# robin-karlsson0/pc-accumulation-lib

Hardware: AMD Instinct MI355X
Metric: Mpoints/s projected+accumulated and BEV frames/s @256x256; 1/2/4/8 GPU (higher is better)
Workload: dtype f64; 1 GPU; KITTI-360 single forward cam, 120k pts/frame, 200 m horizon (~201 live frames, 5169634 stored pts), one 256x256x21 BEV per integrated frame; points_per_frame=120000, bev_px=256, view_m=80

## Files before the change

pc-accumulation-lib_amd/csrc/pca_api.hip:

```cpp
#include <stdio.h>
#include <cmath>
#include "pca_common.h"

__global__ __launch_bounds__(256) void pca_fetch_block_kernel(const uint4 *src, uint4 *dst, int64_t n16)
{
    for (int64_t i = (int64_t)blockIdx.x * 256 + threadIdx.x; i < n16; i += (int64_t)gridDim.x * 256) dst[i] = src[i];
}

int pca_fetch_block(pca_ctx *ctx, const void *mapped_host, int64_t offset, void *dev, int64_t bytes, hipStream_t s)
{
    if (bytes <= 0) return 0;
    void *src = nullptr;
    PCA_CHECK(ctx, hipHostGetDevicePointer(&src, const_cast<void *>(mapped_host), 0));
    src = reinterpret_cast<char *>(src) + offset;
    const int64_t n16 = (bytes + 15) / 16;
    const int grid = (int)((n16 + 255) / 256 < 64 ? (n16 + 255) / 256 : 64);
    hipLaunchKernelGGL(pca_fetch_block_kernel, dim3(grid), dim3(256), 0, s, reinterpret_cast<const uint4 *>(src),
                       reinterpret_cast<uint4 *>(dev), n16);
    PCA_CHECK(ctx, hipGetLastError());
    return 0;
}

int pca_ctx_reserve_tiles(pca_ctx *ctx, int64_t tiles, hipStream_t s)
{
// ... 87 lines not shown
            double Mr[6], Mt[2];
            for (int r = 0; r < 2; ++r) {
                for (int c = 0; c < 3; ++c) Mr[3 * r + c] = now[4 * r] * inv[c] + now[4 * r + 1] * inv[3 + c] + now[4 * r + 2] * inv[6 + c];
                Mt[r] = now[4 * r + 3] - (Mr[3 * r] * m[3] + Mr[3 * r + 1] * m[7] + Mr[3 * r + 2] * m[11]);
            }
            const double tx = Mt[0] - prm->origin[0], ty = Mt[1] - prm->origin[1];
            q[0] = prm->R[0] * tx + prm->R[1] * ty + prm->dx;
            q[1] = prm->R[3] * tx + prm->R[4] * ty + prm->dy;
            for (int c = 0; c < 3; ++c) {
                Q[c] = prm->R[0] * Mr[c] + prm->R[1] * Mr[3 + c];
                Q[3 + c] = prm->R[3] * Mr[c] + prm->R[4] * Mr[3 + c];
            }
        }
        for (int k = 0; k < 6; ++k) if (!std::isfinite(Q[k])) return true;
        if (!std::isfinite(q[0]) || !std::isfinite(q[1])) return true;
        for (int axis = 0; axis < 2; ++axis)
            for (int side = 0; side < 2; ++side) {
                const double s = side ? -1.0 : 1.0;
                const double *row = Q + 3 * axis;
                if (cone) {
                    const double ua = s * (row[0] * cone[0] + row[1] * cone[1] + row[2] * cone[2] + q[axis]);
                    bool out = ua >= h;
                    for (int k = 0; k < 4 && out; ++k) {
                        const double *d = cone + 3 + 3 * k;
                        out = s * (row[0] * d[0] + row[1] * d[1] + row[2] * d[2]) >= 0.0;
                    }
                    if (out) return false;
                }
                if (box) {
                    const float *b = box + 6 * (size_t)f;
                    if (b[0] <= b[1] && b[2] <= b[3] && b[4] <= b[5]) {
                        double lo = s * q[axis];
                        for (int c = 0; c < 3; ++c) {
                            const double x0 = s * row[c] * (double)b[2 * c], x1 = s * row[c] * (double)b[2 * c + 1];
                            lo += x0 < x1 ? x0 : x1;
                        }
                        if (lo >= h) return false;
                    }
                }
            }
        return true;
    };
    int a = 0, b = F - 1;
    while (a <= b && !visible(a)) ++a;
    while (b >= a && !visible(b)) --b;
    if (a > b) { *first = -1; *last = -1; } else { *first = a; *last = b; }
    return 0;
}

int pca_bev_view_hint(pca_ctx *ctx, int slot0, int F, const double *then, const float *box, const double *cone, const double now[12],
                      const pca_bev_params *prm)
{
    if (!ctx) return -1;
    int first = 0, last = 0;
    if (pca_host_view_hull(F, then, box, cone, now, prm, &first, &last)) return -1;
    if (first == 0 && last == F - 1) return 0;
    if (first < 0) { first = 0; last = -1; }
    ctx->bin_first = slot0 + first; ctx->bin_end = slot0 + last + 1; ctx->bin_valid = true;
    return 1;
}

int pca_bev_bin_range(pca_ctx *ctx, int slot_first, int slot_last_plus1)
{
    if (!ctx) return -1;
    ctx->bin_first = slot_first; ctx->bin_end = slot_last_plus1; ctx->bin_valid = slot_last_plus1 >= slot_first;
    return 0;
}

static inline bool box_inside(double x, double y, double lo, double hi) { return lo < x && x < hi && lo < y && y < hi; }

int pca_host_ego_to_grid(const double *full, int F, const double R[9], double dx, double dy, double view, int px,
                         double *rows, int32_t *start)
{
    if (F < 2) { if (F == 1 && start) start[0] = 0; return 0; }
    const double h = 0.5 * view, lo = -h, pxd = (double)px, half_px = 0.5 * pxd;
    auto rot = [&](const double *p, double &x, double &y, double &z) {
        x = fma(R[2], p[2], fma(R[1], p[1], R[0] * p[0])) + dx;
        y = fma(R[5], p[2], fma(R[4], p[1], R[3] * p[0])) + dy;
        z = fma(R[8], p[2], fma(R[7], p[1], R[6] * p[0]));
    };
    auto emit = [&](int m, double x, double y, double z) {
        rows[3 * m + 0] = floor(x / view * pxd + half_px);
        rows[3 * m + 1] = floor(y / view * pxd + half_px);
        rows[3 * m + 2] = z;
    };
    int m = 0;
    double ax, ay, az, bx, by, bz;
    rot(full, ax, ay, az);
    bool a_in = box_inside(ax, ay, lo, h);
    for (int k = 0; k + 1 < F; ++k) {
        rot(full + 3 * (k + 1), bx, by, bz);
        const bool b_in = box_inside(bx, by, lo, h);
        start[k] = m;
        if (a_in) emit(m++, ax, ay, az);
        if (a_in != b_in) {
            double x0 = ax, y0 = ay, x1 = bx, y1 = by, xm = 0.0, ym = 0.0, gap = __builtin_huge_val();
            while (gap > 1e-4) {
                xm = 0.5 * (x0 + x1);
                ym = 0.5 * (y0 + y1);
                const bool p0_in = box_inside(x0, y0, lo, h), mid_in = box_inside(xm, ym, lo, h);
                if (mid_in == p0_in) { gap = sqrt((xm - x0) * (xm - x0) + (ym - y0) * (ym - y0)); x0 = xm; y0 = ym; }
                else { gap = sqrt((xm - x1) * (xm - x1) + (ym - y1) * (ym - y1)); x1 = xm; y1 = ym; }
            }
            emit(m++, xm, ym, az);
        }
        ax = bx; ay = by; az = bz; a_in = b_in;
// ... 131 lines not shown
```

pc-accumulation-lib_amd/csrc/pca_bev.hip:

```cpp
#include "pca_bev_common.h"
#include "pca_k1_body.h"
#include <cstdlib>
#include <mutex>

#define KEY_INVALID 0xffffffffu
#define TS 8
#define TCELLS (TS * TS)
#define NFK (2 * TCELLS)
#ifndef AB_THREADS
#define AB_THREADS 1024
#endif
#define MAX_G 512
#ifndef BIN_RUNR
#define BIN_RUNR 4
#endif
#ifndef BIN_WPE
#define BIN_WPE 4
#endif
#ifndef BIN_UNR
#define BIN_UNR 4
#endif
#ifndef BIN_REG_P
#define BIN_REG_P 12
#endif
#ifndef C_THREADS
#define C_THREADS 256
#endif
#define C_WAVES (C_THREADS / 64)
#define C_HIST_WAVES 4
#define RGB_CAP 4096
#define CONTIG_MIN 2560
#define HEAVY_MIN_DEFAULT 2560
#define FLAG_ROAD (1u << 24)
#define FLAG_DYNOBJ (1u << 25)

struct __attribute__((aligned(16))) RecF { double z; uint32_t iw; uint32_t cw; };
struct RecD { double z; double inten; uint32_t c; uint32_t fk; };

struct alignas(16) BevArgs {
    pca_store st;
    const double *intensity64;
    const int64_t *frame_off;
    int slot_begin, slot_split, slot_end;
    int64_t max_points;
    pca_bev_params prm;
    int n_pend;
    int write_back;
    int pend_slot_end[PCA_BEV_MAX_CHAIN];
    Mat34 pend_T[PCA_BEV_MAX_CHAIN];
    int tx, T, G;
    int Gr, Gp;
    int tile_mult;
    int heavy_min;
    int stagger;
    uint32_t *key;
    uint32_t *bh;
    uint32_t *boff;
    int Gk;
    int bin_first, bin_end;
    int k1_slot, k1_n;
    uint32_t *bh0;
    int split;
    uint32_t *heavy_hint;
    uint32_t heavy_hint_known;
    uint32_t *span_hint;
    uint32_t span_hint_known;
    int heavy_launched;
    uint32_t *heavy;
    void *recs;
    double *planes;
    uint16_t *planes_f16;
    double *extra;
    uint32_t *status;
    int dbg;
};
#define HQ_CLASSES 32
#define HQ_CURSOR 32
#define HQ_DONE 33
#define HQ_IDS 64

struct Window { int64_t lo, hi, sp, c_lo, c_hi; };

__device__ __forceinline__ int chunk_index(const BevArgs &a, int64_t lo, int64_t sp, int64_t chunk)
{
    (void)a; (void)lo; (void)sp; (void)chunk;
    return (int)blockIdx.x;
}
#define K1_SEG 4096
#define K1_RIDE 32
__device__ __forceinline__ int64_t window_end(const BevArgs &a)
{
    const int e = a.Gk ? a.k1_slot : a.slot_end;
    return a.frame_off[a.bin_end < e ? a.bin_end : e];
}
__device__ __forceinline__ int64_t window_begin(const BevArgs &a) { return a.frame_off[a.bin_first]; }
__device__ __forceinline__ Window chunk_of(const BevArgs &a, int &g)
{
    Window w;
    w.lo = window_begin(a);
    const int64_t hi0 = window_end(a);
    w.sp = (a.Gk && a.slot_split > a.k1_slot) ? hi0 : a.frame_off[a.slot_split];
    w.hi = (hi0 - w.lo > a.max_points) ? w.lo + a.max_points : hi0;
    const int G = a.G - a.Gk;
    const int64_t chunk = (w.hi - w.lo + G - 1) / G;
    g = chunk_index(a, w.lo, w.sp, chunk);
    const int c = g - a.Gk;
    w.c_lo = w.lo + (int64_t)c * chunk;
    w.c_hi = w.c_lo + chunk < w.hi ? w.c_lo + chunk : w.hi;
    if (w.c_lo > w.hi) w.c_lo = w.c_hi = w.hi;
    return w;
}
__host__ __device__ __forceinline__ int64_t seg_stride(int64_t n, int G) { return (n + G - 1) / G; }
__device__ __forceinline__ bool bev_split(const BevArgs &a, int64_t window_points)
{
    return a.split == 2 || (a.split == 1 && window_points <= (int64_t)(a.G - a.Gk) * BIN_REG_P * AB_THREADS);
}
__device__ __forceinline__ int table_pos(const BevArgs &a, int g) { return a.Gp ? (g & 7) * a.Gp + (g >> 3) : g; }
__device__ __forceinline__ int table_group(const BevArgs &a, int p)
{
    if (!a.Gp) return p;
// ... 796 lines not shown
        const uint32_t other = dpp_or<0xb1>(0u, val);
        if (ok && !upper) L.S.med2[set][cell][ch] = val + other;
    }
}

__device__ __forceinline__ void wave_cells_hist(TileLds &L, const uint32_t *s_rgb)
{
    const int lane = threadIdx.x & 63, wave = threadIdx.x >> 6;
    if (wave >= C_HIST_WAVES) return;
    uint32_t *h = &L.whist[wave][0][0][0];
    for (int i = 0; i < TCELLS / C_HIST_WAVES; ++i) {
        const int cell = C_HIST_WAVES * i + wave;
        const uint32_t n_p = L.S.cnt[2 * cell], n_f = L.S.cnt[2 * cell + 1], n = n_p + n_f;
        if (n <= 64) continue;
        for (int k = lane; k < 2 * 3 * 128 / 4; k += 64) reinterpret_cast<uint4 *>(h)[k] = make_uint4(0, 0, 0, 0);
        const uint32_t base = L.off[2 * cell];
        for (uint32_t i0 = 0; i0 < n; i0 += 64) {
            const uint32_t idx = i0 + lane;
            const bool act = idx < n;
            const uint32_t v = act ? s_rgb[base + idx] : 0u;
            const uint32_t set = idx >= n_p ? 1u : 0u;
            const uint32_t tag = act ? (v | (set << 24)) : 0xffffffffu;
            const uint32_t first = __builtin_amdgcn_readfirstlane(tag);
            const uint64_t actm = __ballot(act);
            if (__ballot(tag == first) == actm && first != 0xffffffffu) {
                if (lane == (int)__ffsll((unsigned long long)actm) - 1) {
#pragma unroll
                    for (int ch = 0; ch < 3; ++ch)
                        hist16_add(&L.whist[wave][set][ch][0], (v >> (8 * ch)) & 255u, (uint32_t)__popcll(actm));
                }
            } else if (act) {
#pragma unroll
                for (int ch = 0; ch < 3; ++ch) hist16_add(&L.whist[wave][set][ch][0], (v >> (8 * ch)) & 255u, 1u);
            }
        }
#pragma unroll
        for (int ch = 0; ch < 3; ++ch) hist16_medians(L.S, &L.whist[wave][0][ch][0], &L.whist[wave][1][ch][0], cell, ch, n_p, n_f);
    }
}

template <bool I64, int NT>
__device__ __forceinline__ void tile_cell_medians32(TileStats &S, uint32_t (*hist)[256], const RecMap &M, const BevArgs &a, int cell,
                                                    uint32_t r_lo, uint32_t r_hi);

template <bool I64>
__device__ __forceinline__ void cells_drain(const BevArgs &a, TileLds &L, unsigned char *s_buf, bool pushed)
{
    TileStats &S = L.S;
    if (a.heavy_launched) return;
    __shared__ uint32_t s_drain_n;
    if (threadIdx.x == 0) {
        uint32_t n = 0;
        if (pushed) __threadfence();
        if (__hip_atomic_fetch_add(&a.heavy[HQ_DONE], 1u, __ATOMIC_RELAXED, __HIP_MEMORY_SCOPE_AGENT) == gridDim.x - 1) {
            __threadfence();
            for (int c = 0; c < HQ_CLASSES; ++c) n += __hip_atomic_load(&a.heavy[c], __ATOMIC_RELAXED, __HIP_MEMORY_SCOPE_AGENT);
            if (a.heavy_hint && n != a.heavy_hint_known) *a.heavy_hint = n;
        }
        s_drain_n = n;
    }
    __syncthreads();
    if (s_drain_n == 0) return;
    __threadfence();
    const bool extra = a.extra != nullptr;
    const bool div255 = !I64 && a.prm.intensity_div255;
    RecMap &M = *reinterpret_cast<RecMap *>(s_buf);
    uint32_t (*hist)[256] = reinterpret_cast<uint32_t (*)[256]>(s_buf + ((sizeof(RecMap) + 15) & ~(size_t)15));
    static_assert(((sizeof(RecMap) + 15) & ~(size_t)15) + 3 * 256 * 4 <= RGB_CAP * 4, "RecMap + histograms live in the colour buffer");
    for (int cls = 0; cls < HQ_CLASSES; ++cls) {
        const uint32_t n_cls = __hip_atomic_load(&a.heavy[cls], __ATOMIC_RELAXED, __HIP_MEMORY_SCOPE_AGENT);
        for (uint32_t k = 0; k < n_cls; ++k) {
            const int tile = (int)__hip_atomic_load(&a.heavy[HQ_IDS + (size_t)cls * a.T + k], __ATOMIC_RELAXED, __HIP_MEMORY_SCOPE_AGENT);
            __syncthreads();
            stats_init(S, C_THREADS);
            const uint32_t r_hi = recmap_build(M, a, tile, C_THREADS);
            Run run;
            run_reset(run, RUN_NONE);
            const uint32_t per_thread = (r_hi + C_THREADS - 1) / C_THREADS;
            const uint32_t t_lo = threadIdx.x * per_thread, t_hi = t_lo + per_thread < r_hi ? t_lo + per_thread : r_hi;
            for (uint32_t r = t_lo; r < t_hi; ++r) {
                uint32_t kk, c;
                double z, iv;
                load_rec<I64>(a, recmap_at(M, a.Gr, r), kk, c, z, iv);
                if (kk != run.key) {
                    if (run.key != RUN_NONE) run_flush(S, extra, run);
                    run_reset(run, kk);
                }
                run_add(run, extra, c, z, iv, div255);
            }
            if (run.key != RUN_NONE) run_flush(S, extra, run);
            __syncthreads();
            uint32_t *h16 = &L.whist[0][0][0][0];
            for (int c0 = 0; c0 < TCELLS; c0 += 4) {
                uint32_t any = 0;
                for (int c = c0; c < c0 + 4; ++c) any += S.cnt[2 * c] + S.cnt[2 * c + 1];
                if (any == 0) continue;
                for (int k = threadIdx.x; k < 8 * 3 * 128 / 4; k += C_THREADS) reinterpret_cast<uint4 *>(h16)[k] = make_uint4(0, 0, 0, 0);
                __syncthreads();
                for (uint32_t r = threadIdx.x; r < r_hi; r += C_THREADS) {
                    uint32_t kk, v;
                    load_rec_key_colour<I64>(a, recmap_at(M, a.Gr, r), kk, v);
                    const uint32_t rel = kk - 2u * (uint32_t)c0;
                    if (rel >= 8u) continue;
#pragma unroll
                    for (int ch = 0; ch < 3; ++ch) hist16_add(h16 + (rel * 3 + ch) * 128, (v >> (8 * ch)) & 255u, 1u);
                }
                __syncthreads();
// ... 346 lines not shown
    __device__ __forceinline__ void operator()(const float4 (&p)[PPT], const uint32_t (&packed)[PPT], const uint64_t (&km)[PPT]) const
    {
        extern __shared__ uint32_t s_lds[];
        __shared__ uint32_t s_wsum[AB_THREADS / 64];
        __shared__ uint32_t s_dyn[8];
        const int64_t lo = window_begin(a), hi0 = window_end(a);
        const bool split = bev_split(a, hi0 - lo > a.max_points ? a.max_points : hi0 - lo);
        const int hs = split ? 6 : 7, n_hist = split ? 2 * a.T : a.T;
        uint32_t *s_h = s_lds, *s_cur = s_lds + n_hist;
        if (threadIdx.x < 8) {
            uint32_t w = (uint32_t)a.prm.dynobj_mask[0];
#pragma unroll
            for (int i = 1; i < 8; ++i) w = (int)threadIdx.x == i ? (uint32_t)(a.prm.dynobj_mask[i >> 1] >> (32 * (i & 1))) : w;
            s_dyn[threadIdx.x] = w;
        }
        for (int t = threadIdx.x; t < n_hist; t += AB_THREADS) s_h[t] = 0;
        __syncthreads();
        const ViewConst vc = view_const(a);
        const uint32_t set = a.k1_slot >= a.slot_split ? 1u : 0u;
        const int lane = threadIdx.x & 63;
        uint32_t rkey[PPT];
#pragma unroll
        for (int r = 0; r < PPT; ++r) {
            const bool kept = (km[r] >> lane) & 1ull;
            rkey[r] = view_key_lean(vc, (double)p[r].x, (double)p[r].y, (double)p[r].z, kept, set);
            if (rkey[r] != KEY_INVALID) atomicAdd(&s_h[rkey[r] >> hs], 1u);
        }
        __syncthreads();
        bin_scan_tables(a, s_h, s_cur, s_wsum, split, (int)blockIdx.x);
        __syncthreads();
        const uint32_t seg = (uint32_t)blockIdx.x * K1_SEG;
#pragma unroll
        for (int r = 0; r < PPT; ++r) {
            if (rkey[r] == KEY_INVALID) continue;
            const uint32_t pos = seg + atomicAdd(&s_cur[rkey[r] >> hs], 1u);
            bin_store<false>(a, s_dyn, pos, rkey[r], packed[r], (double)p[r].z, 0.0, p[r].w);
        }
    }
};
static_assert(K1_SEG == 1024 * 4, "a K1 piece holds one 1024 x 4 tile");
__global__ __launch_bounds__(AB_THREADS) __attribute__((amdgpu_waves_per_eu(BIN_WPE, BIN_WPE))) void bev_tile_bin_k1(const BevArgs a, const K1Args k)
{
    if ((int)blockIdx.x < a.Gk) k1_body<AB_THREADS, 4, false, false, false>(k, BinK1Tail{a});
    else bev_tile_bin_body<false>(a);
}

template <bool I64>
__global__ __launch_bounds__(AB_THREADS) __attribute__((amdgpu_waves_per_eu(BIN_WPE, BIN_WPE))) void bev_tile_bin(const BevArgs a) { bev_tile_bin_body<I64>(a); }
#if C_THREADS == 512
#define C_OCC __attribute__((amdgpu_waves_per_eu(6, 6)))
#else
#define C_OCC
#endif
template <bool I64>
__global__ __launch_bounds__(C_THREADS) C_OCC void bev_tile_cells(const BevArgs a) { bev_tile_cells_body<I64>(a); }
template <bool I64, bool EXTRA, bool OWN>
__global__ __launch_bounds__(H_THREADS) void bev_tile_cells_heavy(const BevArgs a) { bev_tile_cells_heavy_body<I64, EXTRA, OWN>(a); }
#define PCA_BEV_MANY_MAX 48
__constant__ BevArgs g_bev_many[PCA_BEV_MANY_MAX];
template <bool I64>
__global__ __launch_bounds__(AB_THREADS) __attribute__((amdgpu_waves_per_eu(BIN_WPE, BIN_WPE))) void bev_tile_bin_many()
{
    const BevArgs &a = g_bev_many[blockIdx.y];
    if ((int)blockIdx.x < a.G) bev_tile_bin_body<I64>(a);
}
template <bool I64>
__global__ __launch_bounds__(C_THREADS) C_OCC void bev_tile_cells_many()
{
    bev_tile_cells_body<I64>(g_bev_many[blockIdx.y]);
}
template <bool I64>
__global__ __launch_bounds__(H_THREADS) void bev_tile_cells_heavy_many()
{
    bev_tile_cells_heavy_body<I64, false, false>(g_bev_many[blockIdx.y]);
}

int pca_k1_prepare_pending(pca_ctx *ctx, K1Args *out, int *n_tiles, hipStream_t s);
void pca_k1_pending_launched(pca_ctx *ctx, hipStream_t s);
static inline int64_t align256(int64_t v) { return (v + 255) & ~255ll; }
static inline int tiles_x(int px) { return (px + TS - 1) / TS; }
static inline int max_groups()
{
    const char *e = getenv("PCA_BEV_G");
    const int max_g = e ? atoi(e) : MAX_G;
    return (max_g < 1 || max_g > 1024) ? MAX_G : max_g;
}
static inline int n_groups(int64_t max_points)
{
    const char *c = getenv("PCA_BEV_CHUNK");
    const int max_g = max_groups();
    int per_g = c ? atoi(c) : 8192;
    if (per_g < 1024) per_g = 8192;
    int64_t g = (max_points + per_g - 1) / per_g;
    return (int)(g < 1 ? 1 : (g > max_g ? max_g : g));
}

extern "C" {

int64_t pca_bev_workspace_bytes(int64_t max_points, int px)
{
    if (max_points < 1) max_points = 1;
    const int64_t T = (int64_t)tiles_x(px) * tiles_x(px), G = n_groups(max_points);
    return align256(max_points * 4) + 3 * align256((G + K1_RIDE + 8) * T * 4) + align256((HQ_IDS + HQ_CLASSES * T) * 4) +
           align256((max_points + G + K1_RIDE + K1_SEG) * 24) + 512;
}

int pca_bev_generate(pca_ctx *ctx, const pca_store *store, const double *intensity64, const int64_t *frame_off,
                     int slot_begin, int slot_split, int slot_end, int64_t max_points, const pca_bev_params *prm,
// ... 38 lines not shown
        ctx->err = "bev: R must be a rotation about the z axis (R[2] = R[5] = R[6] = R[7] = 0, R[8] = 1)";
        return -1;
    }
    if (!(slot_begin <= slot_split && slot_split <= slot_end)) { ctx->err = "bev: need slot_begin <= slot_split <= slot_end"; return -1; }
    if (max_points >= (1ll << 32)) { ctx->err = "bev: window too large for 32-bit positions"; return -1; }
    if (workspace_bytes < pca_bev_workspace_bytes(max_points, prm->px)) { ctx->err = "bev: workspace too small"; return -1; }
    a.st = *store;
    a.intensity64 = intensity64;
    a.frame_off = frame_off;
    a.slot_begin = slot_begin; a.slot_split = slot_split; a.slot_end = slot_end;
    a.max_points = max_points;
    a.prm = *prm;
    a.n_pend = n_pending;
    a.write_back = write_back ? 1 : 0;
    for (int k = 0; k < PCA_BEV_MAX_CHAIN; ++k) {
        a.pend_slot_end[k] = slot_begin;
        for (int i = 0; i < 12; ++i) a.pend_T[k].m[i] = 0.0;
        if (k >= n_pending) continue;
        if (pending_slot_ends[k] > slot_end) { ctx->err = "bev: a pending slot end lies beyond the window"; return -1; }
        if (k > 0 && pending_slot_ends[k] < pending_slot_ends[k - 1]) { ctx->err = "bev: pending slot ends must ascend"; return -1; }
        a.pend_slot_end[k] = pending_slot_ends[k];
        for (int i = 0; i < 12; ++i) a.pend_T[k].m[i] = pending_Ts[16 * k + i];
    }
    a.tx = tiles_x(prm->px);
    a.T = a.tx * a.tx;
    a.G = n_groups(max_points);
    bev_table_order(a);
    char *w = reinterpret_cast<char *>((reinterpret_cast<uintptr_t>(workspace) + 255) & ~(uintptr_t)255);
    a.key = reinterpret_cast<uint32_t *>(w); w += align256(max_points * 4);
    a.bh = reinterpret_cast<uint32_t *>(w); w += align256((int64_t)(a.G + K1_RIDE + 8) * a.T * 4);
    a.boff = reinterpret_cast<uint32_t *>(w); w += align256((int64_t)(a.G + K1_RIDE + 8) * a.T * 4);
    a.bh0 = reinterpret_cast<uint32_t *>(w); w += align256((int64_t)(a.G + K1_RIDE + 8) * a.T * 4);
    a.split = 0;
    a.Gk = 0; a.k1_slot = -1; a.k1_n = 0;
    a.bin_first = slot_begin; a.bin_end = slot_end;
    a.heavy = reinterpret_cast<uint32_t *>(w); w += align256((int64_t)(HQ_IDS + HQ_CLASSES * (int64_t)a.T) * 4);
    a.recs = w;
    a.planes = planes;
    a.planes_f16 = planes_f16;
    a.extra = extra_planes;
    { static int hm = -1; if (hm < 0) { const char *e = getenv("PCA_BEV_HEAVY_MIN"); hm = e ? atoi(e) : HEAVY_MIN_DEFAULT; if (hm < 1 || hm > RGB_CAP) hm = RGB_CAP; } a.heavy_min = hm; }
    { static int dbg = -1; if (dbg < 0) { const char *e = getenv("PCA_BEV_DBG"); dbg = e ? atoi(e) : 0; } a.dbg = dbg; }
    { static int sg = -1; if (sg < 0) { const char *e = getenv("PCA_BEV_STAGGER"); sg = e ? atoi(e) : 0; if (sg < 0 || sg > 64) sg = 0; } a.stagger = sg; }
    a.status = ctx->ticket + 1;
    {
        auto gcd = [](int x, int y) { while (y) { const int t = x % y; x = y; y = t; } return x; };
        const int Tp = (a.tx & 3) == 0 ? a.T / 4 : a.T;
        int m = (int)(Tp * 0.6180339887) | 1;
        while (m > 1 && gcd(m, Tp) != 1) m -= 2;
        a.tile_mult = m < 1 ? 1 : m;
    }
    a.heavy_hint = nullptr; a.heavy_hint_known = 0; a.heavy_launched = 1;
    a.span_hint = nullptr; a.span_hint_known = 0;
    return 0;
}

static int bev_set_lds_attributes(pca_ctx *ctx)
{
    static bool lds_set = false;
    if (lds_set) return 0;
#define PCA_BEV_LDS_ATTR(k, bytes) PCA_CHECK(ctx, hipFuncSetAttribute(reinterpret_cast<const void *>(&(k)), hipFuncAttributeMaxDynamicSharedMemorySize, (int)(bytes)))
#define PCA_BEV_HEAVY_ATTR(I) PCA_BEV_LDS_ATTR((bev_tile_cells_heavy<I, false, false>), HEAVY_LDS_BYTES); PCA_BEV_LDS_ATTR((bev_tile_cells_heavy<I, false, true>), HEAVY_LDS_BYTES); \
    PCA_BEV_LDS_ATTR((bev_tile_cells_heavy<I, true, false>), HEAVY_LDS_BYTES); PCA_BEV_LDS_ATTR((bev_tile_cells_heavy<I, true, true>), HEAVY_LDS_BYTES)
    PCA_BEV_HEAVY_ATTR(false);
    PCA_BEV_HEAVY_ATTR(true);
#undef PCA_BEV_HEAVY_ATTR
    PCA_BEV_LDS_ATTR(bev_tile_cells_heavy_many<false>, HEAVY_LDS_BYTES);
    PCA_BEV_LDS_ATTR(bev_tile_cells_heavy_many<true>, HEAVY_LDS_BYTES);
    PCA_BEV_LDS_ATTR(bev_tile_bin_k1, 80 * 1024);
    PCA_BEV_LDS_ATTR(bev_tile_bin<false>, 128 * 1024);
    PCA_BEV_LDS_ATTR(bev_tile_bin<true>, 128 * 1024);
    PCA_BEV_LDS_ATTR(bev_tile_bin_many<false>, 128 * 1024);
    PCA_BEV_LDS_ATTR(bev_tile_bin_many<true>, 128 * 1024);
#undef PCA_BEV_LDS_ATTR
    lds_set = true;
    return 0;
}

int pca_bev_generate_chain(pca_ctx *ctx, const pca_store *store, const double *intensity64, const int64_t *frame_off,
                           int slot_begin, int slot_split, int slot_end, int64_t max_points, const pca_bev_params *prm,
                           const double *pending_Ts, const int *pending_slot_ends, int n_pending, int write_back,
                           void *workspace, int64_t workspace_bytes, double *planes, uint16_t *planes_f16,
                           double *extra_planes, void *stream)
{
    if (!ctx) return -1;
    const bool bin_given = ctx->bin_valid;
    const int bin_first = ctx->bin_first, bin_end = ctx->bin_end;
    ctx->bin_valid = false;
    if (max_points < 1) max_points = 1;
    hipStream_t s = (hipStream_t)stream;
    PCA_CHECK(ctx, hipSetDevice(ctx->device));
    BevArgs a;
    if (bev_prepare(ctx, store, intensity64, frame_off, slot_begin, slot_split, slot_end, max_points, prm, pending_Ts,
                    pending_slot_ends, n_pending, write_back, workspace, workspace_bytes, planes, planes_f16, extra_planes, a))
        return -1;
    if (bev_set_lds_attributes(ctx)) return -1;
    const int heavy_grid = a.T < ctx->n_cu ? a.T : ctx->n_cu;
    a.heavy_hint = ctx->heavy_hint_dev;
    a.heavy_hint_known = *ctx->heavy_hint;
    if (a.heavy_hint_known != 0) ctx->heavy_cooldown = 64;
    else if (ctx->heavy_cooldown > 0) --ctx->heavy_cooldown;
    a.heavy_launched = a.heavy_hint_known != 0 || ctx->heavy_cooldown > 0;
    { static int always = -1; if (always < 0) { const char *e = getenv("PCA_BEV_HEAVY_ALWAYS"); always = e ? atoi(e) : 0; } if (always) a.heavy_launched = 1; }
    { static int sp = -1; if (sp < 0) { const char *e = getenv("PCA_BEV_SPLIT"); sp = e ? atoi(e) : 1; }
      a.split = (sp && a.heavy_launched && !intensity64 && (size_t)a.T * 16 <= 128 * 1024) ? (sp == 2 ? 2 : 1) : 0; }
    const size_t lds = (size_t)a.T * 8 * (a.split ? 2 : 1);
    int one_round = 0;
    if (bin_given) {
        static int cu = -1;
        static int64_t pts = -1;
        if (cu < 0) { const char *e = getenv("PCA_BEV_CULL"); cu = e ? atoi(e) : 1; }
        if (pts < 0) { const char *e = getenv("PCA_BEV_ONE_ROUND_PTS"); pts = e ? atoll(e) : 14500; }
        if (cu && !(n_pending > 0 && write_back)) {
            int f = bin_first > slot_begin ? bin_first : slot_begin, e = bin_end < slot_end ? bin_end : slot_end;
            if (e < f) e = f;
            a.bin_first = f; a.bin_end = e;
            a.span_hint = ctx->heavy_hint_dev + 1;
            a.span_hint_known = ctx->heavy_hint[1];
            if (pts > 0 && a.span_hint_known != 0 && (int64_t)a.span_hint_known * 1024 <= pts * ctx->n_cu && a.G > ctx->n_cu) one_round = ctx->n_cu;
        }
    }
    bool fuse = false;
    K1Args k1a;
    if (ctx->k1_pend.valid) {
        static int fk = -1;
        if (fk < 0) { const char *e = getenv("PCA_FUSE_K1"); fk = e ? atoi(e) : 1; }
        const pca_ctx::K1Pending &pd = ctx->k1_pend;
        int nt = 0;
        bool owed_ok = true;
        for (int k = 0; k < n_pending; ++k) owed_ok = owed_ok && pending_slot_ends[k] <= pd.slot;
        fuse = fk && owed_ok && !intensity64 && pd.stream == s && pd.slot == slot_end - 1 && pd.slot >= slot_begin && pd.frame_off == frame_off &&
               pd.store.x == store->x && lds <= 80 * 1024 && pd.fr.n <= K1_RIDE * K1_SEG && pd.fr.n <= max_points &&
               pca_k1_prepare_pending(ctx, &k1a, &nt, s) == 0 && nt <= K1_RIDE;
        { static int fd = -1; if (fd < 0) { const char *e = getenv("PCA_FUSE_DBG"); fd = e ? atoi(e) : 0; }
          if (fd && !fuse)
              fprintf(stderr, "bev: K1 of slot %d not taken along: switch %d owed_ok %d i64 %d stream %d slot %d (window %d..%d) frame_off %d store %d lds %zu n %d max_points %lld nt %d\n",
                      pd.slot, fk, (int)owed_ok, intensity64 != nullptr, pd.stream == s, pd.slot == slot_end - 1, slot_begin, slot_end,
                      pd.frame_off == frame_off, pd.store.x == store->x, lds, pd.fr.n, (long long)max_points, nt); }
        if (fuse) {
            const int cap = max_groups(), G0 = a.G;
            if (one_round) one_round -= nt;
            a.G = one_round > 0 ? one_round + nt : (G0 + nt <= cap || (cap - 2 * nt) * 4 < 3 * G0) ? G0 + nt : cap - nt;
            a.Gk = nt; bev_table_order(a); a.k1_slot = pd.slot; a.k1_n = pd.fr.n;
            a.max_points = max_points - pd.fr.n;
        }
        else if (pca_k1_flush_pending(ctx)) return -1;
    }
    if (one_round > 0 && !fuse) { a.G = one_round; bev_table_order(a); }
    if (ctx->profiling == 2) pca_prof_begin(ctx, PCA_K_BEV_UNIT, s);
#define PCA_BEV_HEAVY_LAUNCH(I, E, O) PCA_LAUNCH_SHM(ctx, PCA_K_BEV_CELLS_HEAVY, (bev_tile_cells_heavy<I, E, O>), dim3(heavy_grid), dim3(H_THREADS), HEAVY_LDS_BYTES, s, a)
#define PCA_BEV_HEAVY_PICK(I)                                                                                          \
    do {                                                                                                               \
        if (a.extra) { if (a.split) PCA_BEV_HEAVY_LAUNCH(I, true, true); else PCA_BEV_HEAVY_LAUNCH(I, true, false); }  \
        else { if (a.split) PCA_BEV_HEAVY_LAUNCH(I, false, true); else PCA_BEV_HEAVY_LAUNCH(I, false, false); }        \
    } while (0)
    if (intensity64) {
        PCA_LAUNCH_SHM(ctx, PCA_K_BEV_BIN, bev_tile_bin<true>, dim3(a.G), dim3(AB_THREADS), lds, s, a);
        PCA_LAUNCH(ctx, PCA_K_BEV_CELLS, bev_tile_cells<true>, dim3(a.T), dim3(C_THREADS), s, a);
        if (a.heavy_launched) PCA_BEV_HEAVY_PICK(true);
    } else {
        if (fuse) {
            PCA_LAUNCH_SHM(ctx, PCA_K_BEV_BIN, bev_tile_bin_k1, dim3(a.G), dim3(AB_THREADS), lds, s, a, k1a);
            pca_k1_pending_launched(ctx, s);
        } else {
            PCA_LAUNCH_SHM(ctx, PCA_K_BEV_BIN, bev_tile_bin<false>, dim3(a.G), dim3(AB_THREADS), lds, s, a);
        }
        PCA_LAUNCH(ctx, PCA_K_BEV_CELLS, bev_tile_cells<false>, dim3(a.T), dim3(C_THREADS), s, a);
        if (a.heavy_launched) PCA_BEV_HEAVY_PICK(false);
    }
#undef PCA_BEV_HEAVY_PICK
#undef PCA_BEV_HEAVY_LAUNCH
    if (ctx->profiling == 2) pca_prof_end(ctx, s);
    PCA_CHECK(ctx, hipGetLastError());
    return 0;
}

int pca_bev_generate_many(pca_ctx *ctx, const pca_store *store, const double *intensity64, const int64_t *frame_off,
                          const pca_bev_job *jobs, int n_jobs, int64_t max_points, void *workspace,
                          int64_t workspace_bytes, void *stream)
{
    if (!ctx) return -1;
    if (pca_k1_flush_pending(ctx)) return -1;
    ctx->bin_valid = false;
    if (!jobs || n_jobs < 1) { ctx->err = "bev: bad job list"; return -1; }
    if (n_jobs > 65535) { ctx->err = "bev: at most 65535 rasters per call"; return -1; }
    if (max_points < 1) max_points = 1;
    hipStream_t s = (hipStream_t)stream;
    PCA_CHECK(ctx, hipSetDevice(ctx->device));
    const int px = jobs[0].prm.px;
    const int64_t per = (pca_bev_workspace_bytes(max_points, px) + 255) & ~255ll;
    if (workspace_bytes < per * n_jobs + 256) { ctx->err = "bev: workspace too small for this many rasters"; return -1; }
    const int64_t up_bytes = (int64_t)sizeof(BevArgs) * n_jobs;
    if (ctx->bevm_busy) { PCA_CHECK(ctx, hipEventSynchronize(ctx->bevm_ev)); ctx->bevm_busy = false; }
    if (up_bytes > ctx->bevm_cap) {
        if (ctx->bevm_pin) PCA_CHECK(ctx, hipHostFree(ctx->bevm_pin));
        ctx->bevm_pin = nullptr; ctx->bevm_cap = 0;
        PCA_CHECK(ctx, hipHostMalloc(&ctx->bevm_pin, (size_t)(2 * up_bytes), hipHostMallocMapped));
        ctx->bevm_cap = 2 * up_bytes;
    }
    if (!ctx->bevm_ev) PCA_CHECK(ctx, hipEventCreateWithFlags(&ctx->bevm_ev, hipEventDisableTiming));
    BevArgs *ha = reinterpret_cast<BevArgs *>(ctx->bevm_pin);
    char *ws = reinterpret_cast<char *>((reinterpret_cast<uintptr_t>(workspace) + 255) & ~(uintptr_t)255);
    int G = 0, T = 0;
    for (int k = 0; k < n_jobs; ++k) {
        const pca_bev_job &j = jobs[k];
        if (j.prm.px != px) { ctx->err = "bev: the rasters of one call share the grid size"; return -1; }
        if (bev_prepare(ctx, store, intensity64, frame_off, j.slot_begin, j.slot_split, j.slot_end, max_points, &j.prm, nullptr,
                        nullptr, 0, 1, ws + per * k, per, j.planes, j.planes_f16, nullptr, ha[k]))
            return -1;
        G = ha[k].G; T = ha[k].T;
    }
    if (bev_set_lds_attributes(ctx)) return -1;
    const size_t lds = (size_t)T * 8;
    const int heavy_grid = T < 8 ? T : 8;
    static std::mutex many_mutex;
    static hipEvent_t many_last[64] = {};
    std::lock_guard<std::mutex> many_lock(many_mutex);
    hipEvent_t &last = many_last[ctx->device & 63];
    if (last) PCA_CHECK(ctx, hipStreamWaitEvent(s, last, 0));
    else PCA_CHECK(ctx, hipEventCreateWithFlags(&last, hipEventDisableTiming));
// ... 74 lines not shown
```

pc-accumulation-lib_amd/csrc/pca_session.hip:

```cpp
#include <vector>

#include "pca_common.h"

int pca_stage_copy(const void *const *src, void *const *dst, const int64_t *bytes, int n);

static inline int64_t up256(int64_t v) { return (v + 255) & ~255ll; }

extern "C" {

int pca_kitti_integrate(pca_ctx *ctx, const pca_kitti_obs *obs, const double P[12], int H, int W,
                        const uint64_t filter_mask[4], const pca_store *store, int64_t *frame_off, int slot, int sample_mode,
                        pca_host_track *track, const double *T_new_prev, double horizon, int64_t *evicted,
                        double *path_length, void *stream)
{
    if (!ctx) return -1;
    if (!obs || obs->n < 0 || !P || !filter_mask || !store || !frame_off) { ctx->err = "kitti_integrate: bad arguments"; return -1; }
    if (track && (!T_new_prev || !evicted || !path_length)) { ctx->err = "kitti_integrate: the pose track needs T_new_prev and its outputs"; return -1; }
    hipStream_t s = (hipStream_t)stream;
    PCA_CHECK(ctx, hipSetDevice(ctx->device));
    if (pca_k1_flush_pending(ctx)) return -1;
    const void *in[4] = {obs->pts, obs->rgb, obs->sem, obs->sem_gt};
    const int64_t size[4] = {16ll * obs->n, 3ll * H * W, 1ll * H * W, 1ll * obs->n};
    const void *dev[4] = {in[0], in[1], in[2], in[3]};
    int64_t off[4] = {0, 0, 0, 0}, total = 0;
// ... 23 lines not shown
                dev[k] = (char *)st.dev + off[k];
            }
        pca_stage_copy(src, dst, bytes, m);
        static int64_t side_min = -1;
        if (side_min < 0) { const char *e = getenv("PCA_H2D_SIDE_MIN"); side_min = e ? atoll(e) : (256ll << 10); }
        if (total >= side_min) {
            if (!ctx->h2d_stream[0]) PCA_CHECK(ctx, hipStreamCreateWithFlags(&ctx->h2d_stream[0], hipStreamNonBlocking));
            if (!ctx->h2d_done[0]) PCA_CHECK(ctx, hipEventCreateWithFlags(&ctx->h2d_done[0], hipEventDisableTiming));
            PCA_CHECK(ctx, hipMemcpyAsync(st.dev, st.pin, (size_t)total, hipMemcpyHostToDevice, ctx->h2d_stream[0]));
            PCA_CHECK(ctx, hipEventRecord(ctx->h2d_done[0], ctx->h2d_stream[0]));
            PCA_CHECK(ctx, hipStreamWaitEvent(s, ctx->h2d_done[0], 0));
        } else {
            PCA_CHECK(ctx, hipMemcpyAsync(st.dev, st.pin, (size_t)total, hipMemcpyHostToDevice, s));
        }
        slot_st = &st;
    }
    pca_kitti_frame fr;
    fr.pts = (const float *)dev[0]; fr.rgb = (const uint8_t *)dev[1]; fr.sem = (const uint8_t *)dev[2];
    fr.sem_gt = (const uint8_t *)dev[3]; fr.n = obs->n; fr.reserved = 0;
    const bool plain = obs->n > 0 && sample_mode == PCA_SAMPLE_NEAREST && (fr.sem_gt || ((int64_t)H * W * 3 >= 4 && fr.rgb && fr.sem)) &&
                       obs->n <= (1 << 20);
    if (ctx->k1_defer && plain) {
        pca_ctx::K1Pending &pd = ctx->k1_pend;
        pd.fr = fr;
        for (int i = 0; i < 12; ++i) pd.P[i] = P[i];
        pd.H = H; pd.W = W;
        for (int i = 0; i < 4; ++i) pd.filt[i] = filter_mask[i];
        pd.store = *store; pd.frame_off = frame_off; pd.slot = slot; pd.sample_mode = sample_mode; pd.stream = s;
        pd.stage_idx = slot_st ? (int)(slot_st - ctx->stage) : -1;
        pd.valid = true;
    } else {
        const int rc = pca_kitti_project_sample_filter_ex(ctx, &fr, 1, P, H, W, filter_mask, store, frame_off, slot, sample_mode, stream);
        if (slot_st) {
            const hipError_t e = hipEventRecord(slot_st->done, s);
            if (e == hipSuccess) slot_st->busy = true;
            else {
                (void)hipStreamSynchronize(s);
                if (rc == 0) { ctx->err = std::string("kitti_integrate: hipEventRecord(stage done): ") + hipGetErrorString(e); return -1; }
            }
        }
        if (rc != 0) return rc;
    }
    if (track) *evicted = pca_host_track_step(track, T_new_prev, horizon, path_length);
    return 0;
}

int pca_kitti_generate_bev(pca_ctx *ctx, const pca_store *store, const int64_t *frame_off, int slot_begin, int slot_split,
                           int slot_end, int64_t max_points, const pca_bev_params *prm, const double *pending_Ts,
                           const int *pending_slot_ends, int n_pending, int write_back, void *workspace,
                           int64_t workspace_bytes, uint16_t *planes_f16, void *host_planes, const pca_host_track *track,
                           double *traj_rows, int32_t *traj_start, int32_t *n_rows, void *stream)
{
    if (!ctx) return -1;
    if (!prm || !planes_f16 || !track || !traj_rows || !traj_start || !n_rows) { ctx->err = "kitti_generate_bev: bad arguments"; return -1; }
    const int64_t F = pca_host_track_len(track);
    if (F != slot_end - slot_begin) { ctx->err = "kitti_generate_bev: the pose track and the window disagree about the number of frames"; return -1; }
    static thread_local std::vector<double> rel;
    rel.resize((size_t)(3 * (F > 0 ? F : 1)));
    const double *Hp = pca_host_track_poses(track);
    for (int64_t f = 0; f < F; ++f)
        for (int k = 0; k < 3; ++k) rel[(size_t)(3 * f + k)] = Hp[4 * f + k] - prm->origin[k];
    *n_rows = pca_host_ego_to_grid(rel.data(), (int)F, prm->R, prm->dx, prm->dy, prm->view, prm->px, traj_rows, traj_start);
    if (pca_bev_generate_chain(ctx, store, nullptr, frame_off, slot_begin, slot_split, slot_end, max_points, prm, pending_Ts,
                               pending_slot_ends, n_pending, write_back, workspace, workspace_bytes, nullptr, planes_f16,
                               nullptr, stream) != 0)
        return -1;
    if (!host_planes) return 0;
    return pca_host_d2h_async(ctx, planes_f16, host_planes, 21ll * prm->px * prm->px * 2, stream);
}

int pca_kitti_integrate_v(pca_ctx *ctx, pca_kitti_integrate_args *a)
{
    if (!ctx) return -1;
    if (!a) { ctx->err = "kitti_integrate_v: no argument block"; return -1; }
    return pca_kitti_integrate(ctx, a->obs, a->P, a->H, a->W, a->filter_mask, a->store, a->frame_off, a->slot, a->sample_mode,
                               a->track, a->T_new_prev, a->horizon, &a->evicted, &a->path_length, a->stream);
}

int pca_kitti_generate_bev_v(pca_ctx *ctx, pca_kitti_generate_bev_args *a)
{
    if (!ctx) return -1;
    if (!a) { ctx->err = "kitti_generate_bev_v: no argument block"; return -1; }
    a->hinted = 0;
    if (a->hint_F > 0 && !(a->n_pending > 0 && a->write_back)) {
        const int rc = pca_bev_view_hint(ctx, a->hint_slot0, a->hint_F, a->hint_then, a->hint_box, a->hint_cone, a->hint_now, a->prm);
        if (rc < 0) { ctx->err = "kitti_generate_bev_v: bad view hint"; return -1; }
        a->hinted = rc;
    }
    return pca_kitti_generate_bev(ctx, a->store, a->frame_off, a->slot_begin, a->slot_split, a->slot_end, a->max_points, a->prm,
                                  a->pending_Ts, a->pending_slot_ends, a->n_pending, a->write_back, a->workspace,
                                  a->workspace_bytes, a->planes_f16, a->host_planes, a->track, a->traj_rows, a->traj_start,
                                  &a->n_rows, a->stream);
}

}
```

pc-accumulation-lib_amd/pca_amd/device_store.py:

```python
import ctypes as C
import os

import numpy as np
import torch

from . import _lib
from ._lib import PcaBevParams, PcaKittiFrame, PcaStore

CULL = os.environ.get('PCA_BEV_CULL', '1') != '0'


class DeviceStore:
    CHAIN_MAX = 4
    CHAIN_K = int(os.environ.get('PCA_BEV_CHAIN', '4'))

    def __init__(self, capacity=1 << 24, max_frames=4096, device=None, intensity_div255=False):
        self.ctx = _lib.Context.get(device)
        self.device = torch.device('cuda', self.ctx.device_index)
        self.intensity_div255 = bool(intensity_div255)
        self.max_frames = int(max_frames)
        self._alloc(int(capacity))
        self.frame_off = torch.zeros(self.max_frames + 1, dtype=torch.int64, device=self.device)
        self._moved = np.eye(4)
        self.cull = CULL
# ... 61 lines not shown
            M[3] = (0., 0., 0., 1.)
            self._moved = M

    def _note_frame(self, slot, cone_key):
        self._then[slot] = self._moved[:3].reshape(12)
        if cone_key is not None:
            if self._cone is None or self._cone[0] != cone_key:
                if self._cone is not None:
                    self._has_cone[self.head:self.tail] = False
                    self._n_nocone = self.tail - self.head
                out = np.empty(15)
                Pm = np.frombuffer(cone_key[0], dtype=np.float64)
                self.ctx.lib.pca_host_camera_cone(Pm.ctypes.data, int(cone_key[1]), int(cone_key[2]), out.ctypes.data)
                self._cone = (cone_key, out, out.ctypes.data)
            self._has_cone[slot] = True
        else:
            self._n_nocone += 1
        self._since_box += 1
        self._poll_boxes()
        if self._since_box >= self.BOX_EVERY and self._box_copy is None:
            n = self.tail - self.head
            if n > 0:
                if self._box_pin is None or self._box_pin.shape[0] < self.frame_box.shape[0]:
                    self._box_pin = torch.empty(tuple(self.frame_box.shape), dtype=torch.int32, pin_memory=True)
                self._box_pin[:n].copy_(self.frame_box[self.head:self.tail], non_blocking=True)
                ev = torch.cuda.Event()
                ev.record()
                self._box_copy = (ev, self.head, n)
                self._since_box = 0

    def _poll_boxes(self):
        if self._box_copy is None or not self._box_copy[0].query():
            return
        _, first, n = self._box_copy
        self._box_copy = None
        rows = self._box_pin[:n].numpy()
        dec = np.empty((n, 6), dtype=np.float32)
        self.ctx.lib.pca_f32_box_decode(rows.ctypes.data, n, dec.ctypes.data)
        known = dec[:, 0] <= dec[:, 1]
        tgt = self._box[first:first + n]
        tgt[known] = dec[known]

    def view_hint_into(self, args, first_frame, last_frame):
        n = last_frame - first_frame
        if not self.cull or n < 4:
            return 0
        a = self.head + first_frame
        args.hint_slot0 = a
        args.hint_then, args.hint_box = self._then_addr + 96 * a, self._box_addr + 24 * a
        args.hint_cone = self._cone[2] if (self._cone is not None and self._n_nocone == 0) else None
        args.hint_now = self._moved.ctypes.data
        return n

    def view_hint(self, prm, first_frame, last_frame, write_back):
        n = last_frame - first_frame
        if not self.cull or write_back or n < 4:
            return 0
        a = self.head + first_frame
        cone = self._cone[2] if (self._cone is not None and self._n_nocone == 0) else None
        return self._count_hint(self.ctx.lib.pca_bev_view_hint(self.ctx.h, a, n, self._then_addr + 96 * a, self._box_addr + 24 * a, cone,
                                              self._moved.ctypes.data, C.addressof(prm)))

    def _count_hint(self, r):
        self.hints_taken += 1 if r > 0 else 0
        return r

    def c_store(self):
        if self._cstore is None:
            self._cstore = PcaStore(self.x.data_ptr(), self.y.data_ptr(), self.z.data_ptr(), self.intensity.data_ptr(),
                                    self.rgbs.data_ptr(), self.inst.data_ptr(), self.dyn.data_ptr(), self.capacity,
                                    self.frame_box.data_ptr())
        return self._cstore

    @property
    def n_frames(self):
        return self.tail - self.head

    def set_defer_k1(self, on):
        self.ctx.check(self.ctx.lib.pca_k1_defer(self.ctx.h, 1 if on else 0))
        self.ctx.k1_defer = bool(on)
        if not on:
            self._k1_noted = None

    def flush_k1(self):
        if self._k1_noted is not None:
            self.ctx.check(self.ctx.lib.pca_k1_flush(self.ctx.h))
            self._k1_noted = None

    def __del__(self):
        try:
            if self._k1_noted is not None:
                self.flush_k1()
        except Exception:
            pass

    def offsets(self):
        self.flush_k1()
        off = self.frame_off[self.head:self.tail + 1].cpu().numpy()
        self.lb_head = int(off[0])
        self.ub_tail = int(off[-1])
        self._ub = [int(v) for v in np.diff(off)]
        self._ub_sum = sum(self._ub)
        return off

    def sizes(self):
        return np.diff(self.offsets())

    def poll_status(self):
        self.ctx.poll_status()
# ... 223 lines not shown
                                              _lib.f64_array(Ts, Ts.size), Ts.shape[0], ctx.stream()))
        st, ctx = self.c_store(), self.ctx
        ctx.check(ctx.lib.pca_retransform_batch_tail(ctx.h, C.byref(st), self.frame_off.data_ptr(), first_new, n_new,
                                                     _lib.f64_array(Ts, Ts.size), ctx.stream()))

    def flush_pending(self):
        pend, self._pending = self._pending, []
        begin = self.head
        for k, (_, end_slot) in enumerate(pend):
            if end_slot > begin:
                self._launch_retransform(np.stack([T for T, _ in pend[k:]]), begin, end_slot)
                begin = end_slot

    def mark_dynamic(self, pairs):
        pairs = list(pairs)
        if not pairs:
            return
        slots = (C.c_int32 * len(pairs))(*[self.head + int(f) for f, _ in pairs])
        insts = (C.c_int32 * len(pairs))(*[int(i) for _, i in pairs])
        st = self.c_store()
        ctx = self.ctx
        ctx.check(ctx.lib.pca_mark_dynamic(ctx.h, C.byref(st), self.frame_off.data_ptr(), slots, insts, len(pairs),
                                           ctx.stream()))

    def voxel_dedup(self, voxel_size):
        if self.n_frames == 0:
            return
        self.flush_pending()
        ctx, lib = self.ctx, self.ctx.lib
        max_points = self.max_window_points()
        need = lib.pca_voxel_dedup_workspace_bytes(max_points, self.n_frames)
        if self._dedup_ws is None or self._dedup_ws.numel() < need:
            self._dedup_ws = torch.empty(int(need) + 256, dtype=torch.uint8, device=self.device)
        st = self.c_store()
        ctx.check(lib.pca_voxel_dedup(ctx.h, C.byref(st), self.frame_off.data_ptr(), self.head, self.tail,
                                      float(voxel_size), max_points, self._dedup_ws.data_ptr(),
                                      self._dedup_ws.numel(), ctx.stream()))

    def bev(self, split_frame, prm, want_f64=False, intensity64=None, first_frame=0, last_frame=None, out16=None,
            extra=None):
        ctx, lib = self.ctx, self.ctx.lib
        last_frame = self.n_frames if last_frame is None else last_frame
        px = int(prm.px)
        max_points = self.bev_workspace(px)
        if out16 is not None:
            assert out16.dtype == torch.float16 and out16.is_contiguous() and tuple(out16.shape) == (21, px, px)
        p16 = out16 if out16 is not None else torch.empty((21, px, px), dtype=torch.float16, device=self.device)
        p64 = torch.empty((21, px, px), dtype=torch.float64, device=self.device) if want_f64 else None
        st = self.c_store()
        n_pend, pend_T, pend_ends, write_back = self.bev_pending(first_frame, last_frame)
        if extra is not None:
            assert extra.dtype == torch.float64 and extra.is_contiguous() \
                and tuple(extra.shape) == (3, len(_lib.BEV_EXTRA_PLANES), px, px)
        self.view_hint(prm, first_frame, last_frame, n_pend > 0 and write_back)
        ctx.check(lib.pca_bev_generate_chain(ctx.h, C.byref(st), None if intensity64 is None else intensity64.data_ptr(),
                                             self.frame_off.data_ptr(), self.head + first_frame, self.head + split_frame,
                                             self.head + last_frame, max_points, C.byref(prm), pend_T, pend_ends, n_pend,
                                             write_back, self._ws.data_ptr(), self._ws.numel(),
                                             None if p64 is None else p64.data_ptr(), p16.data_ptr(),
                                             None if extra is None else extra.data_ptr(), ctx.stream()))
        self.bev_done(write_back)
        return p16, p64

    def bev_workspace(self, px):
        max_points = self.max_window_points()
        if self._ws is None or max_points > self._ws_points or px != self._ws_px:
            self._ws_points, self._ws_px = int(max_points * 1.25) + 1, px
            need = self.ctx.lib.pca_bev_workspace_bytes(self._ws_points, px)
            if self._ws is None or self._ws.numel() < need:
                self._ws = torch.empty(int(need) + 256, dtype=torch.uint8, device=self.device)
        return max_points

    def bev_pending(self, first_frame, last_frame):
        if not self._pending:
            return 0, None, None, 1
        if first_frame != 0 or self._pending[-1][1] > self.head + last_frame:
            self.flush_pending()
            return 0, None, None, 1
        n_pend = 0
        for T, e in self._pending:
            if e > self.head:
                self._pend_T_np[16 * n_pend:16 * n_pend + 16] = T
                self._pend_ends[n_pend] = int(e)
                n_pend += 1
        if n_pend == 0:
            return 0, None, None, 0
        return n_pend, self._pend_T, self._pend_ends, (1 if n_pend >= self.CHAIN_K else 0)

    def bev_done(self, write_back):
        if self._pending and write_back:
            self._pending = []
        self._k1_noted = None

    def bev_many(self, jobs, out16):
        ctx, lib = self.ctx, self.ctx.lib
        n = len(jobs)
        if n == 0:
            return out16
        self.flush_pending()
        px = int(jobs[0][1].px)
        assert out16.dtype == torch.float16 and out16.is_contiguous() and tuple(out16.shape) == (n, 21, px, px)
        max_points = self.max_window_points()
        per = (int(lib.pca_bev_workspace_bytes(max_points, px)) + 255) & ~255
        need = per * n + 512
        if self._ws_many is None or self._ws_many.numel() < need:
            self._ws_many = torch.empty(int(need * 1.25), dtype=torch.uint8, device=self.device)
        cj = (_lib.PcaBevJob * n)()
# ... 92 lines not shown
```

Measured before the change: 1437 Mpoints/s.

## Allow view-hull culling during write-back by adding tail blocks for owed transforms

View-hull frame culling of the BEV bin range was previously turned off whenever pending pose write-back was owed, because culled frames would miss their deferred coordinate update. The cells kernel now launches extra blocks past the tile count that apply the owed transforms to points outside the binned window. With that in place the view hint can be taken on write-back frames too. The drain counter now compares against the tile count rather than the grid size, and bin_valid is reset on error paths. The cost is extra write-back blocks and more complex index bookkeeping.

```diff
diff --git a/pc-accumulation-lib_amd/csrc/pca_api.hip b/pc-accumulation-lib_amd/csrc/pca_api.hip
--- a/pc-accumulation-lib_amd/csrc/pca_api.hip
+++ b/pc-accumulation-lib_amd/csrc/pca_api.hip
@@ -163,6 +163,7 @@
                       const pca_bev_params *prm)
 {
     if (!ctx) return -1;
+    ctx->bin_valid = false;
     int first = 0, last = 0;
     if (pca_host_view_hull(F, then, box, cone, now, prm, &first, &last)) return -1;
     if (first == 0 && last == F - 1) return 0;
diff --git a/pc-accumulation-lib_amd/csrc/pca_bev.hip b/pc-accumulation-lib_amd/csrc/pca_bev.hip
--- a/pc-accumulation-lib_amd/csrc/pca_bev.hip
+++ b/pc-accumulation-lib_amd/csrc/pca_bev.hip
@@ -66,6 +66,7 @@
     uint32_t *span_hint;
     uint32_t span_hint_known;
     int heavy_launched;
+    int Gw;
     uint32_t *heavy;
     void *recs;
     double *planes;
@@ -968,7 +969,7 @@
     if (threadIdx.x == 0) {
         uint32_t n = 0;
         if (pushed) __threadfence();
-        if (__hip_atomic_fetch_add(&a.heavy[HQ_DONE], 1u, __ATOMIC_RELAXED, __HIP_MEMORY_SCOPE_AGENT) == gridDim.x - 1) {
+        if (__hip_atomic_fetch_add(&a.heavy[HQ_DONE], 1u, __ATOMIC_RELAXED, __HIP_MEMORY_SCOPE_AGENT) == (uint32_t)a.T - 1) {
             __threadfence();
             for (int c = 0; c < HQ_CLASSES; ++c) n += __hip_atomic_load(&a.heavy[c], __ATOMIC_RELAXED, __HIP_MEMORY_SCOPE_AGENT);
             if (a.heavy_hint && n != a.heavy_hint_known) *a.heavy_hint = n;
@@ -1421,8 +1422,48 @@
 #else
 #define C_OCC
 #endif
+#define WB_PTS 4096
+__device__ __forceinline__ void bev_write_back_rest(const BevArgs &a)
+{
+    const int64_t lo0 = a.frame_off[a.slot_begin];
+    PendHi ph;
+    int64_t pe = lo0;
+#pragma unroll
+    for (int k = 0; k < PCA_BEV_MAX_CHAIN; ++k) {
+        ph.v[k] = (k < a.n_pend && a.pend_slot_end[k] > a.slot_begin) ? a.frame_off[a.pend_slot_end[k]] : lo0;
+        pe = ph.v[k] > pe ? ph.v[k] : pe;
+    }
+    const int64_t wlo = window_begin(a), hi0 = window_end(a);
+    const int64_t whi = (hi0 - wlo > a.max_points) ? wlo + a.max_points : hi0;
+    const int64_t a_end = wlo < pe ? wlo : pe, b_lo = whi > lo0 ? whi : lo0;
+    const int64_t nA = a_end > lo0 ? a_end - lo0 : 0, nB = pe > b_lo ? pe - b_lo : 0, n = nA + nB;
+    constexpr int U = 4;
+    const int64_t step = (int64_t)a.Gw * U * C_THREADS;
+    for (int64_t base = (int64_t)((int)blockIdx.x - a.T) * U * C_THREADS + threadIdx.x; base < n; base += step) {
+        double X[U], Y[U], Z[U];
+        int64_t p[U];
+#pragma unroll
+        for (int u = 0; u < U; ++u) {
+            const int64_t i = base + u * C_THREADS;
+            p[u] = i < nA ? lo0 + i : b_lo + (i - nA);
+            const bool in = i < n;
+            X[u] = in ? a.st.x[p[u]] : 0.0;
+            Y[u] = in ? a.st.y[p[u]] : 0.0;
+            Z[u] = in ? a.st.z[p[u]] : 0.0;
+        }
+#pragma unroll
+        for (int u = 0; u < U; ++u) {
+            if (base + u * C_THREADS >= n) continue;
+            if (apply_owed(a, ph, p[u], X[u], Y[u], Z[u])) { a.st.x[p[u]] = X[u]; a.st.y[p[u]] = Y[u]; a.st.z[p[u]] = Z[u]; }
+        }
+    }
+}
 template <bool I64>
-__global__ __launch_bounds__(C_THREADS) C_OCC void bev_tile_cells(const BevArgs a) { bev_tile_cells_body<I64>(a); }
+__global__ __launch_bounds__(C_THREADS) C_OCC void bev_tile_cells(const BevArgs a)
+{
+    if ((int)blockIdx.x >= a.T) { bev_write_back_rest(a); return; }
+    bev_tile_cells_body<I64>(a);
+}
 template <bool I64, bool EXTRA, bool OWN>
 __global__ __launch_bounds__(H_THREADS) void bev_tile_cells_heavy(const BevArgs a) { bev_tile_cells_heavy_body<I64, EXTRA, OWN>(a); }
 #define PCA_BEV_MANY_MAX 48
@@ -1567,6 +1608,7 @@
     }
     a.heavy_hint = nullptr; a.heavy_hint_known = 0; a.heavy_launched = 1;
     a.span_hint = nullptr; a.span_hint_known = 0;
+    a.Gw = 0;
     return 0;
 }
 
@@ -1626,13 +1668,20 @@
         static int64_t pts = -1;
         if (cu < 0) { const char *e = getenv("PCA_BEV_CULL"); cu = e ? atoi(e) : 1; }
         if (pts < 0) { const char *e = getenv("PCA_BEV_ONE_ROUND_PTS"); pts = e ? atoll(e) : 14500; }
-        if (cu && !(n_pending > 0 && write_back)) {
+        if (cu) {
             int f = bin_first > slot_begin ? bin_first : slot_begin, e = bin_end < slot_end ? bin_end : slot_end;
             if (e < f) e = f;
             a.bin_first = f; a.bin_end = e;
             a.span_hint = ctx->heavy_hint_dev + 1;
             a.span_hint_known = ctx->heavy_hint[1];
             if (pts > 0 && a.span_hint_known != 0 && (int64_t)a.span_hint_known * 1024 <= pts * ctx->n_cu && a.G > ctx->n_cu) one_round = ctx->n_cu;
+            int owed_end = slot_begin;
+            for (int k = 0; k < n_pending; ++k) owed_end = pending_slot_ends[k] > owed_end ? pending_slot_ends[k] : owed_end;
+            if (n_pending > 0 && write_back && (f > slot_begin || e < owed_end)) {
+                const int64_t known = (int64_t)a.span_hint_known * 1024, rest = max_points > known ? max_points - known : WB_PTS;
+                const int64_t gw = (rest + WB_PTS - 1) / WB_PTS, gmax = 8ll * ctx->n_cu;
+                a.Gw = (int)(gw < 1 ? 1 : (gw > gmax ? gmax : gw));
+            }
         }
     }
     bool fuse = false;
@@ -1671,7 +1720,7 @@
     } while (0)
     if (intensity64) {
         PCA_LAUNCH_SHM(ctx, PCA_K_BEV_BIN, bev_tile_bin<true>, dim3(a.G), dim3(AB_THREADS), lds, s, a);
-        PCA_LAUNCH(ctx, PCA_K_BEV_CELLS, bev_tile_cells<true>, dim3(a.T), dim3(C_THREADS), s, a);
+        PCA_LAUNCH(ctx, PCA_K_BEV_CELLS, bev_tile_cells<true>, dim3(a.T + a.Gw), dim3(C_THREADS), s, a);
         if (a.heavy_launched) PCA_BEV_HEAVY_PICK(true);
     } else {
         if (fuse) {
@@ -1680,7 +1729,7 @@
         } else {
             PCA_LAUNCH_SHM(ctx, PCA_K_BEV_BIN, bev_tile_bin<false>, dim3(a.G), dim3(AB_THREADS), lds, s, a);
         }
-        PCA_LAUNCH(ctx, PCA_K_BEV_CELLS, bev_tile_cells<false>, dim3(a.T), dim3(C_THREADS), s, a);
+        PCA_LAUNCH(ctx, PCA_K_BEV_CELLS, bev_tile_cells<false>, dim3(a.T + a.Gw), dim3(C_THREADS), s, a);
         if (a.heavy_launched) PCA_BEV_HEAVY_PICK(false);
     }
 #undef PCA_BEV_HEAVY_PICK
diff --git a/pc-accumulation-lib_amd/csrc/pca_session.hip b/pc-accumulation-lib_amd/csrc/pca_session.hip
--- a/pc-accumulation-lib_amd/csrc/pca_session.hip
+++ b/pc-accumulation-lib_amd/csrc/pca_session.hip
@@ -99,9 +99,9 @@
                            double *traj_rows, int32_t *traj_start, int32_t *n_rows, void *stream)
 {
     if (!ctx) return -1;
-    if (!prm || !planes_f16 || !track || !traj_rows || !traj_start || !n_rows) { ctx->err = "kitti_generate_bev: bad arguments"; return -1; }
+    if (!prm || !planes_f16 || !track || !traj_rows || !traj_start || !n_rows) { ctx->bin_valid = false; ctx->err = "kitti_generate_bev: bad arguments"; return -1; }
     const int64_t F = pca_host_track_len(track);
-    if (F != slot_end - slot_begin) { ctx->err = "kitti_generate_bev: the pose track and the window disagree about the number of frames"; return -1; }
+    if (F != slot_end - slot_begin) { ctx->bin_valid = false; ctx->err = "kitti_generate_bev: the pose track and the window disagree about the number of frames"; return -1; }
     static thread_local std::vector<double> rel;
     rel.resize((size_t)(3 * (F > 0 ? F : 1)));
     const double *Hp = pca_host_track_poses(track);
@@ -127,11 +127,11 @@
 int pca_kitti_generate_bev_v(pca_ctx *ctx, pca_kitti_generate_bev_args *a)
 {
     if (!ctx) return -1;
-    if (!a) { ctx->err = "kitti_generate_bev_v: no argument block"; return -1; }
+    if (!a) { ctx->bin_valid = false; ctx->err = "kitti_generate_bev_v: no argument block"; return -1; }
     a->hinted = 0;
-    if (a->hint_F > 0 && !(a->n_pending > 0 && a->write_back)) {
+    if (a->hint_F > 0) {
         const int rc = pca_bev_view_hint(ctx, a->hint_slot0, a->hint_F, a->hint_then, a->hint_box, a->hint_cone, a->hint_now, a->prm);
-        if (rc < 0) { ctx->err = "kitti_generate_bev_v: bad view hint"; return -1; }
+        if (rc < 0) { ctx->bin_valid = false; ctx->err = "kitti_generate_bev_v: bad view hint"; return -1; }
         a->hinted = rc;
     }
     return pca_kitti_generate_bev(ctx, a->store, a->frame_off, a->slot_begin, a->slot_split, a->slot_end, a->max_points, a->prm,
diff --git a/pc-accumulation-lib_amd/pca_amd/device_store.py b/pc-accumulation-lib_amd/pca_amd/device_store.py
--- a/pc-accumulation-lib_amd/pca_amd/device_store.py
+++ b/pc-accumulation-lib_amd/pca_amd/device_store.py
@@ -137,9 +137,9 @@
         args.hint_now = self._moved.ctypes.data
         return n
 
-    def view_hint(self, prm, first_frame, last_frame, write_back):
+    def view_hint(self, prm, first_frame, last_frame):
         n = last_frame - first_frame
-        if not self.cull or write_back or n < 4:
+        if not self.cull or n < 4:
             return 0
         a = self.head + first_frame
         cone = self._cone[2] if (self._cone is not None and self._n_nocone == 0) else None
@@ -469,7 +469,7 @@
         if extra is not None:
             assert extra.dtype == torch.float64 and extra.is_contiguous() \
                 and tuple(extra.shape) == (3, len(_lib.BEV_EXTRA_PLANES), px, px)
-        self.view_hint(prm, first_frame, last_frame, n_pend > 0 and write_back)
+        self.view_hint(prm, first_frame, last_frame)
         ctx.check(lib.pca_bev_generate_chain(ctx.h, C.byref(st), None if intensity64 is None else intensity64.data_ptr(),
                                              self.frame_off.data_ptr(), self.head + first_frame, self.head + split_frame,
                                              self.head + last_frame, max_points, C.byref(prm), pend_T, pend_ends, n_pend,
```

Measured after the change: 1457 Mpoints/s (median of 6 runs). 1.01x the previous value.
